# SmoothKen/knn-svc

Measured on AMD Instinct MI355X. Metric: audio-sec converted/sec (xRT) end-to-end, cold target pool, higher is better.
Workload: dtype f32; 1 GPU; north-star point per rank: 30 s source vs 10 min target pool (20 x 30 s), ckpt_type=mix, post_opt_0.2, cold (pool encoded inside the step); seeded random weights of WavLM-Large (6 layers executed) and the 22.9 M-param generator; nq=1500, np_per_rank=30000, wavlm_batch_chunks=32, pipeline_depth=2

## Files before the change

### knn_svc_amd/csrc/common.h

```cpp
#pragma once
#include <hip/hip_runtime.h>
#include <stdint.h>
#include <stdio.h>
#include <stdarg.h>
#include "../../include/knnsvc_hip.h"

typedef float f32x4 __attribute__((ext_vector_type(4)));
typedef float f32x16 __attribute__((ext_vector_type(16)));

extern thread_local char g_knnsvc_err[512];

static inline int knnsvc_fail(int code, const char* fmt, ...) {
    va_list ap;
    va_start(ap, fmt);
    vsnprintf(g_knnsvc_err, sizeof(g_knnsvc_err), fmt, ap);
    va_end(ap);
    return code;
}

#define KN_REQUIRE(cond, ...) do { if (!(cond)) return knnsvc_fail(KNNSVC_EINVAL, __VA_ARGS__); } while (0)

static inline int knnsvc_check_launch(const char* what) {
    hipError_t e = hipGetLastError();
    if (e != hipSuccess) return knnsvc_fail(KNNSVC_EHIP, "%s: %s", what, hipGetErrorString(e));
// ... 30 lines not shown
    if (n_voices < 2 || n_voices > KNNSVC_BLEND_MAX_VOICES)
        return knnsvc_fail(KNNSVC_EINVAL, "%s: n_voices %d outside 2..%d", entry, (int)n_voices, KNNSVC_BLEND_MAX_VOICES);
    if (!host_weights) return knnsvc_fail(KNNSVC_EINVAL, "%s: null weight table", entry);
    out->nv = n_voices;
    for (int s = 0; s < KNNSVC_MAX_SEGMENTS; ++s)
        for (int v = 0; v < KNNSVC_BLEND_MAX_VOICES; ++v) out->w[s][v] = 0.0;
    for (int s = 0; s < n_seg; ++s) {
        double sum = 0.0;
        bool positive = false;
        for (int v = 0; v < n_voices; ++v) {
            const double a = host_weights[(size_t)s * n_voices + v];
            if (!(a >= 0.0 && a <= 1.79769313486231570815e308))
                return knnsvc_fail(KNNSVC_EINVAL, "%s: segment %d: weight %d is %g, not finite and >= 0", entry, s, v, a);
            positive = positive || a > 0.0;
            sum += a;
            out->w[s][v] = a;
        }
        if (!positive) return knnsvc_fail(KNNSVC_EINVAL, "%s: segment %d: no positive weight", entry, s);
        if (!(sum - 1.0 <= 1e-6 && 1.0 - sum <= 1e-6))
            return knnsvc_fail(KNNSVC_EINVAL, "%s: segment %d: the weights sum to %.9g, not 1 (the caller normalises)", entry, s, sum);
    }
    return KNNSVC_OK;
}

struct KnBlendRow { double w[KNNSVC_BLEND_MAX_VOICES]; int live; };
__device__ __forceinline__ KnBlendRow kn_blend_row(const KnBlendWeights& bw, int s) {
    KnBlendRow r;
    r.live = 0;
#pragma unroll
    for (int v = 0; v < KNNSVC_BLEND_MAX_VOICES; ++v) {
        r.w[v] = v < bw.nv ? bw.w[s][v] : 0.0;
        if (r.w[v] != 0.0) ++r.live;
    }
    return r;
}
__device__ __forceinline__ float kn_blend_mix(const KnBlendRow& r, const float (&x)[KNNSVC_BLEND_MAX_VOICES]) {
#pragma clang fp contract(off)
    double acc = 0.0;
    float one = 0.f;
    bool first = true;
#pragma unroll
    for (int v = 0; v < KNNSVC_BLEND_MAX_VOICES; ++v) {
        if (r.w[v] != 0.0) {
            const double p = r.w[v] * (double)x[v];
            acc = first ? p : acc + p;
            first = false;
            one = x[v];
        }
    }
    return r.live == 1 ? one : (float)acc;
}

bool knnsvc_match_generic_k();

template <auto KERNEL>
static inline int kn_lds_optin(int bytes, const char* entry) {
    static int granted = 0;
    if (bytes <= granted) return KNNSVC_OK;
    if (hipFuncSetAttribute((const void*)KERNEL, hipFuncAttributeMaxDynamicSharedMemorySize, bytes) != hipSuccess)
        return knnsvc_fail(KNNSVC_EHIP, "%s: hipFuncSetAttribute failed", entry);
    granted = bytes;
    return KNNSVC_OK;
}

template <int WN, int TM, int TN>
struct Acc32 {
    __device__ __forceinline__ static int acc_row(int wave, int lane, int i, int r) {
        return (wave / WN) * TM * 32 + i * 32 + (r & 3) + 8 * (r >> 2) + 4 * (lane >> 5);
    }
    __device__ __forceinline__ static int acc_col(int wave, int lane, int j) {
        return (wave % WN) * TN * 32 + j * 32 + (lane & 31);
    }
};

#define KN_ZERO_ACC(ACC, TM, TN, NR)                                                                            \
    _Pragma("unroll") for (int i = 0; i < (TM); ++i)                                                           \
        _Pragma("unroll") for (int j = 0; j < (TN); ++j)                                                       \
            _Pragma("unroll") for (int r = 0; r < (NR); ++r) ACC[i][j][r] = 0.f;

namespace {
__global__ __launch_bounds__(256) void kn_zero_kernel(unsigned* __restrict__ p, long n) {
    const long i = (long)blockIdx.x * 256 + threadIdx.x;
    if (i < n) p[i] = 0u;
}
}
static inline int kn_zero_async(void* p, size_t bytes, hipStream_t st) {
    const long n = (long)(bytes / 4);
    if (n == 0) return KNNSVC_OK;
    hipLaunchKernelGGL(kn_zero_kernel, dim3((unsigned)((n + 255) / 256)), dim3(256), 0, st, (unsigned*)p, n);
    return knnsvc_check_launch("zero_fill");
}

__device__ __forceinline__ float kn_gelu(float x) {
#ifdef KN_GELU_ERFF
    return 0.5f * x * (1.0f + erff(x * 0.70710678118654752440f));
#else
#pragma clang fp contract(off)
    const float z = fabsf(x) * 0.70710678118654752440f;
    const float t = __builtin_amdgcn_rcpf(fmaf(0.39f, z, 1.0f));
    float p = -0.1137684788031453f;
    p = fmaf(p, t, 0.4433318425354039f);
    p = fmaf(p, t, -0.3176995829519751f);
    p = fmaf(p, t, 0.32477925011974735f);
    p = fmaf(p, t, 0.045694387408764885f);
    p = fmaf(p, t, 0.11766258084307574f);
    p *= t;
// ... 72 lines not shown
```

### knn_svc_amd/csrc/elementwise.hip

```cpp
#include "common.h"
#include <cstdlib>
#include "gemm2_core.h"

namespace {

__device__ __forceinline__ void store_split4(float* row, int c, f32x4 y) {
    g2_u32x2 hi, lo;
    f16x2_split4(y, KN_F16X2_A_SCALE, hi, lo);
    char* ob = (char*)row + (c >> 5) * 128 + (c & 31) * 2;
    *(g2_u32x2*)ob = hi;
    *(g2_u32x2*)(ob + 64) = lo;
}
__device__ __forceinline__ f32x4 load_split4(const float* row, int c) {
    const char* ib = (const char*)row + (c >> 5) * 128 + (c & 31) * 2;
    const g2_u32x2 hi = *(const g2_u32x2*)ib, lo = *(const g2_u32x2*)(ib + 64);
    f32x4 y;
#pragma unroll
    for (int e = 0; e < 4; ++e) {
        const unsigned short hb = (unsigned short)(hi[e >> 1] >> (16 * (e & 1))), lb = (unsigned short)(lo[e >> 1] >> (16 * (e & 1)));
        y[e] = ((float)__builtin_bit_cast(_Float16, hb) + (float)__builtin_bit_cast(_Float16, lb)) * (1.0f / KN_F16X2_A_SCALE);
    }
    return y;
}

__device__ __forceinline__ float gelu_erf(float v) {
#pragma clang fp contract(off)
    return kn_gelu(v);
}

template <int MAXV, int R>
__global__ __launch_bounds__(256) void layernorm_kernel(const float* __restrict__ x, long rows, int dim, int ldx,
                                                       const float* __restrict__ gamma, const float* __restrict__ beta,
                                                       int gelu, float* __restrict__ out, int ldo) {
#pragma clang fp contract(off)
    const int lane = threadIdx.x & 63;
    const long row0 = ((long)blockIdx.x * 4 + (threadIdx.x >> 6)) * R;
    if (row0 >= rows) return;
    f32x4 v[R][MAXV];
    float s[R];
#pragma unroll
    for (int r = 0; r < R; ++r) {
        s[r] = 0.f;
        const bool ok = row0 + r < rows;
        const float* xr = x + (row0 + r) * (long)ldx;
#pragma unroll
        for (int i = 0; i < MAXV; ++i) {
            const int c = lane * 4 + 256 * i;
            if (ok && c < dim) { v[r][i] = *(const f32x4*)(xr + c); s[r] += (v[r][i][0] + v[r][i][1]) + (v[r][i][2] + v[r][i][3]); }
            else v[r][i] = (f32x4){0.f, 0.f, 0.f, 0.f};
        }
    }
    float mean[R], q[R];
#pragma unroll
    for (int r = 0; r < R; ++r) mean[r] = wave_sum(s[r]) / (float)dim;
#pragma unroll
    for (int r = 0; r < R; ++r) {
        q[r] = 0.f;
#pragma unroll
        for (int i = 0; i < MAXV; ++i) {
            const int c = lane * 4 + 256 * i;
            if (c < dim) {
#pragma unroll
                for (int e = 0; e < 4; ++e) { const float d = v[r][i][e] - mean[r]; q[r] = fmaf(d, d, q[r]); }
            }
        }
    }
#pragma unroll
    for (int r = 0; r < R; ++r) {
        const float var = wave_sum(q[r]) / (float)dim;
        const float rstd = 1.0f / sqrtf(var + 1e-5f);
        if (row0 + r >= rows) continue;
        float* orow = out + (row0 + r) * (long)ldo;
#pragma unroll
        for (int i = 0; i < MAXV; ++i) {
            const int c = lane * 4 + 256 * i;
            if (c < dim) {
                const f32x4 g = *(const f32x4*)(gamma + c), b = *(const f32x4*)(beta + c);
                f32x4 y;
#pragma unroll
                for (int e = 0; e < 4; ++e) {
                    float t = fmaf((v[r][i][e] - mean[r]) * rstd, g[e], b[e]);
                    y[e] = (gelu & 1) ? gelu_erf(t) : t;
                }
                if (gelu & 2) store_split4(orow, c, y);
                else *(f32x4*)(orow + c) = y;
            }
        }
    }
}

template <int CPL, int KMAXT, int RP>
__global__ __launch_bounds__(256) void conv0_ln_gelu_kernel(const float* __restrict__ x, long L, long T, int k, int stride,
                                                           const float* __restrict__ w, const float* __restrict__ gamma,
                                                           const float* __restrict__ beta, float* __restrict__ out, int split, int subs) {
    __shared__ float xs[2][64 * 8 + 32];
    const int lane = threadIdx.x & 63, wave = threadIdx.x >> 6;
    const int C = CPL * 64;
    const long b = blockIdx.y;
    const float* xb = x + b * L;
    const int span = 63 * stride + k;
    constexpr int NP = (CPL + 1) / 2;
    f32x2 wr[NP][KMAXT], g[NP], be[NP];
#pragma unroll
    for (int c = 0; c < NP; ++c) {
        const int ch = lane * CPL + 2 * c, ch1 = CPL > 1 ? ch + 1 : ch;
        g[c] = (f32x2){gamma[ch], gamma[ch1]}; be[c] = (f32x2){beta[ch], beta[ch1]};
#pragma unroll
        for (int t = 0; t < KMAXT; ++t) wr[c][t] = t < k ? (f32x2){w[ch * k + t], w[ch1 * k + t]} : (f32x2){0.f, 0.f};
    }
  for (int sub = 0; sub < subs; ++sub) {
    const long m0 = ((long)blockIdx.x * subs + sub) * 64;
    if (m0 >= T) break;
    float* xsb = xs[sub & 1];
    for (int i = threadIdx.x; i < span; i += 256) {
        const long p = m0 * stride + i;
        xsb[i] = p < L ? xb[p] : 0.f;
    }
    __syncthreads();
    for (int r = 0; r < 16; r += RP) {
        f32x2 y[RP][NP];
        float s[RP], mean[RP], q[RP], rstd[RP];
#pragma unroll
        for (int u = 0; u < RP; ++u) {
            const int lm = wave * 16 + r + u;
            float xv[KMAXT];
#pragma unroll
            for (int t = 0; t < KMAXT; ++t) xv[t] = t < k ? xsb[lm * stride + t] : 0.f;
            s[u] = 0.f;
#pragma unroll
            for (int c = 0; c < NP; ++c) {
                f32x2 a = {0.f, 0.f};
#pragma unroll
                for (int t = 0; t < KMAXT; ++t) a = __builtin_elementwise_fma(wr[c][t], (f32x2)(xv[t]), a);
                y[u][c] = a; s[u] += a[0]; if (CPL > 1) s[u] += a[1];
            }
        }
#pragma unroll
        for (int u = 0; u < RP; ++u) mean[u] = (RP > 1 ? wave_sum_dpp(s[u]) : wave_sum(s[u])) / (float)C;
#pragma unroll
        for (int u = 0; u < RP; ++u) {
            q[u] = 0.f;
#pragma unroll
            for (int c = 0; c < CPL; ++c) { const float d = y[u][c >> 1][c & 1] - mean[u]; q[u] += d * d; }
        }
#pragma unroll
        for (int u = 0; u < RP; ++u) rstd[u] = 1.0f / sqrtf((RP > 1 ? wave_sum_dpp(q[u]) : wave_sum(q[u])) / (float)C + 1e-5f);
#pragma unroll
        for (int u = 0; u < RP; ++u) {
            const long m = m0 + wave * 16 + r + u;
            if (m >= T) break;
            float* o = out + (b * T + m) * C + lane * CPL;
#pragma unroll
            for (int c = 0; c < NP; ++c) y[u][c] = kn_gelu2(__builtin_elementwise_fma((y[u][c] - mean[u]) * rstd[u], g[c], be[c]));
            if (CPL % 4 == 0) {
                if (split) {
                    float* orow = out + (b * T + m) * C;
#pragma unroll
                    for (int c = 0; c < CPL; c += 4) store_split4(orow, lane * CPL + c, (f32x4){y[u][c / 2][0], y[u][c / 2][1], y[u][c / 2 + 1][0], y[u][c / 2 + 1][1]});
                } else {
#pragma unroll
                    for (int c = 0; c < CPL; c += 4) *(f32x4*)(o + c) = (f32x4){y[u][c / 2][0], y[u][c / 2][1], y[u][c / 2 + 1][0], y[u][c / 2 + 1][1]};
                }
            } else {
#pragma unroll
                for (int c = 0; c < CPL; ++c) o[c] = y[u][c >> 1][c & 1];
            }
        }
    }
  }
}

__global__ __launch_bounds__(256) void gate_kernel(const float* __restrict__ xn, long rows, int heads, int ldx,
                                                  const float* __restrict__ w2, const float* __restrict__ b2,
                                                  const float* __restrict__ grep_a, float* __restrict__ gate, int split) {
    const int lane = threadIdx.x & 63;
    const long row = (long)blockIdx.x * 4 + (threadIdx.x >> 6);
    if (row >= rows) return;
    const int h = lane >> 2, part = lane & 3;
    float sa = 0.f, sb = 0.f;
    if (h < heads) {
        const float* xr = xn + row * (long)ldx + lane * 16;
#pragma unroll
        for (int e = 0; e < 16; e += 4) {
            const f32x4 xv = split ? load_split4(xn + row * (long)ldx, lane * 16 + e) : *(const f32x4*)(xr + e);
            const f32x4 wa = *(const f32x4*)(w2 + part * 16 + e), wb = *(const f32x4*)(w2 + 64 + part * 16 + e);
#pragma unroll
            for (int t = 0; t < 4; ++t) { sa += xv[t] * wa[t]; sb += xv[t] * wb[t]; }
        }
    }
    sa += __shfl_xor(sa, 1, 64); sa += __shfl_xor(sa, 2, 64);
    sb += __shfl_xor(sb, 1, 64); sb += __shfl_xor(sb, 2, 64);
    if (h < heads && part == 0) {
        const float ga = 1.0f / (1.0f + expf(-(sa + b2[0])));
        const float gb = 1.0f / (1.0f + expf(-(sb + b2[1])));
        gate[row * heads + h] = ga * (gb * grep_a[h] - 1.0f) + 2.0f;
    }
}

__global__ __launch_bounds__(256) void weighted_gather_kernel(const long* __restrict__ idx, const float* __restrict__ w,
                                                             long nq, int k, const float* __restrict__ pool, int dim,
                                                             int ld, int mean_mode, float* __restrict__ out) {
#pragma clang fp contract(off)
    const long row = blockIdx.x;
    const bool mean = !w && mean_mode == 1;
    for (int c = threadIdx.x; c < dim; c += 256) {
        float acc = 0.f;
        for (int j = 0; j < k; ++j) {
            const float wj = w ? w[row * k + j] : 1.0f / (float)k;
            const float x = pool[idx[row * k + j] * (long)ld + c];
            const float t = mean ? x : x * wj;
            acc = j == 0 ? t : acc + t;
        }
        out[row * (long)dim + c] = mean ? acc / (float)k : acc;
    }
}

__global__ void reflect_pad_kernel(const float* __restrict__ x, long n, int pad, float* __restrict__ out) {
    const long i = (long)blockIdx.x * blockDim.x + threadIdx.x;
    if (i >= n + 2 * (long)pad) return;
    long j = i - pad;
    if (j < 0) j = -j;
    if (j >= n) j = 2 * (n - 1) - j;
// ... 74 lines not shown
    for (int o = 32; o > 0; o >>= 1) mx = fmaxf(mx, __shfl_xor(mx, o, 64));
    const float f = f0[t];
    for (int k = lane + 1; k <= n_harm; k += 64) {
        float v;
        if (f == 0.f) v = k == 1 ? mx : 0.f;
        else {
            const int nb = bins * 8;
            float pos = ((f * (float)k) * 2.0f) * (float)nb / 16000.0f;
            pos = fminf(pos, (float)nb);
            const int gi = (int)rintf(pos);
            if (gi >= nb) v = 0.f;
            else {
                float src = ((float)gi + 0.5f) * 0.125f - 0.5f;
                if (src < 0.f) src = 0.f;
                const int i0 = (int)src;
                const int i1 = i0 + (i0 < bins - 1 ? 1 : 0);
                const float l1 = src - (float)i0, l0 = 1.0f - l1;
                v = l0 * s[i0] + l1 * s[i1];
            }
        }
        harm[t * n_harm + (k - 1)] = 0.0108f * v;
    }
}

__global__ __launch_bounds__(256) void mask_rows_kernel(float* __restrict__ x, int T, int dim, int ld, const int* __restrict__ lens) {
    const int b = blockIdx.y;
    const int len = lens[b];
    const long n4 = (long)(T - len) * (dim / 4);
    for (long i = (long)blockIdx.x * blockDim.x + threadIdx.x; i < n4; i += (long)gridDim.x * blockDim.x) {
        const long r = len + i / (dim / 4); const int c = (int)(i % (dim / 4)) * 4;
        *(f32x4*)(x + ((long)b * T + r) * ld + c) = (f32x4){0.f, 0.f, 0.f, 0.f};
    }
}

}

extern "C" int knnsvc_mask_rows(float* x, int32_t batches, int32_t T, int32_t dim, int32_t ld, const int32_t* lens, void* stream) {
    KN_REQUIRE(x && lens && batches > 0 && batches <= 65535 && T > 0 && dim > 0 && dim % 4 == 0 && ld >= dim && ld % 4 == 0 &&
               ((uintptr_t)x & 15) == 0, "mask_rows: bad arguments");
    hipLaunchKernelGGL(mask_rows_kernel, dim3(64, (unsigned)batches), dim3(256), 0, (hipStream_t)stream, x, T, dim, ld, lens);
    return knnsvc_check_launch("mask_rows");
}

extern "C" int knnsvc_layernorm(const float* x, int64_t rows, int32_t dim, int32_t ldx, const float* gamma,
                                const float* beta, int32_t gelu, float* out, int32_t ldo, void* stream) {
    KN_REQUIRE(x && gamma && beta && out, "layernorm: null pointer");
    KN_REQUIRE(dim > 0 && dim % 4 == 0 && dim <= 2048, "layernorm: dim must be a multiple of 4 and <= 2048");
    KN_REQUIRE(ldx % 4 == 0 && ldo % 4 == 0 && ldx >= dim && ldo >= dim, "layernorm: bad row strides");
    KN_REQUIRE(!(gelu & 2) || (dim % 32 == 0 && ldo % 32 == 0), "layernorm: split output needs dim % 32 == 0 and ldo % 32 == 0");
    KN_REQUIRE(((uintptr_t)x & 15) == 0 && ((uintptr_t)out & 15) == 0 && ((uintptr_t)gamma & 15) == 0 &&
               ((uintptr_t)beta & 15) == 0, "layernorm: pointers must be 16-byte aligned");
    if (rows <= 0) return KNNSVC_OK;
    hipStream_t st = (hipStream_t)stream;
    if (dim <= 512)
        hipLaunchKernelGGL((layernorm_kernel<2, 4>), dim3((unsigned)cdiv64(rows, 16)), dim3(256), 0, st, x, (long)rows, dim, ldx,
                           gamma, beta, gelu, out, ldo);
    else if (dim <= 1024)
        hipLaunchKernelGGL((layernorm_kernel<4, 2>), dim3((unsigned)cdiv64(rows, 8)), dim3(256), 0, st, x, (long)rows, dim, ldx,
                           gamma, beta, gelu, out, ldo);
    else
        hipLaunchKernelGGL((layernorm_kernel<8, 1>), dim3((unsigned)cdiv64(rows, 4)), dim3(256), 0, st, x, (long)rows, dim, ldx,
                           gamma, beta, gelu, out, ldo);
    return knnsvc_check_launch("layernorm");
}

extern "C" int knnsvc_wavlm_gate(const float* xn, int64_t rows, int32_t heads, int32_t head_dim, int32_t ldx,
                                 const float* w2, const float* b2, const float* grep_a, float* gate, int32_t x_f16x2, void* stream) {
    KN_REQUIRE(xn && w2 && b2 && grep_a && gate, "wavlm_gate: null pointer");
    KN_REQUIRE(head_dim == 64 && heads >= 1 && heads <= 16, "wavlm_gate: head_dim must be 64, heads <= 16");
    KN_REQUIRE(ldx % 4 == 0 && ldx >= heads * 64 && ((uintptr_t)xn & 15) == 0 && ((uintptr_t)w2 & 15) == 0,
               "wavlm_gate: alignment");
    if (rows <= 0) return KNNSVC_OK;
    hipLaunchKernelGGL(gate_kernel, dim3((unsigned)cdiv64(rows, 4)), dim3(256), 0, (hipStream_t)stream,
                       xn, (long)rows, heads, ldx, w2, b2, grep_a, gate, x_f16x2);
    return knnsvc_check_launch("wavlm_gate");
}

extern "C" int knnsvc_weighted_gather(const int64_t* idx, const float* w, int64_t nq, int32_t k, const float* pool,
                                      int32_t dim, int32_t ld, int32_t mean_mode, float* out, void* stream) {
    KN_REQUIRE(idx && pool && out && k > 0 && dim > 0 && ld >= dim, "weighted_gather: bad arguments");
    KN_REQUIRE(mean_mode == 0 || mean_mode == 1, "weighted_gather: mean_mode %d is neither 0 nor 1", (int)mean_mode);
    if (nq <= 0) return KNNSVC_OK;
    hipLaunchKernelGGL(weighted_gather_kernel, dim3((unsigned)nq), dim3(256), 0, (hipStream_t)stream,
                       (const long*)idx, w, (long)nq, k, pool, dim, ld, mean_mode, out);
    return knnsvc_check_launch("weighted_gather");
}

extern "C" int knnsvc_reflect_pad(const float* x, int64_t n, int32_t pad, float* out, void* stream) {
    KN_REQUIRE(x && out && n > pad && pad >= 0, "reflect_pad: needs n > pad >= 0");
    const long tot = n + 2 * (long)pad;
    hipLaunchKernelGGL(reflect_pad_kernel, dim3((unsigned)cdiv64(tot, 256)), dim3(256), 0, (hipStream_t)stream,
                       x, (long)n, pad, out);
    return knnsvc_check_launch("reflect_pad");
}

extern "C" int knnsvc_reflect_pad_batch(const float* x, const int64_t* offs, int32_t batches, int32_t pad, float* out,
                                        int64_t stride, void* stream) {
    KN_REQUIRE(x && offs && out && batches > 0 && batches <= 65535 && pad >= 0 && stride > 2 * (int64_t)pad,
               "reflect_pad_batch: bad arguments (every item needs n > pad; stride > 2 pad)");
    const unsigned gx = (unsigned)(cdiv64(stride, 256) < 2048 ? cdiv64(stride, 256) : 2048);
    hipLaunchKernelGGL(reflect_pad_batch_kernel, dim3(gx, (unsigned)batches), dim3(256), 0, (hipStream_t)stream,
                       x, (const long*)offs, pad, out, (long)stride);
    return knnsvc_check_launch("reflect_pad_batch");
}

extern "C" int knnsvc_spec_harm(const float* reim, int64_t rows, int32_t bins, int32_t ld, const float* f0, int32_t n_harm,
                                float* spec, float* harm, void* stream) {
    KN_REQUIRE(reim && f0 && spec && harm && bins > 0 && bins <= 4096 && ld >= 2 * bins && n_harm > 0, "spec_harm: bad arguments");
    if (rows <= 0) return KNNSVC_OK;
    hipLaunchKernelGGL(spec_harm_kernel, dim3((unsigned)cdiv64(rows, 4)), dim3(256), (size_t)4 * bins * sizeof(float),
                       (hipStream_t)stream, reim, (long)rows, bins, ld, f0, n_harm, spec, harm);
    return knnsvc_check_launch("spec_harm");
}

extern "C" int knnsvc_complex_mag(const float* reim, int64_t rows, int32_t bins, int32_t ld, float* out, void* stream) {
    KN_REQUIRE(reim && out && bins > 0 && ld >= 2 * bins, "complex_mag: bad arguments");
    if (rows <= 0) return KNNSVC_OK;
    hipLaunchKernelGGL(complex_mag_kernel, dim3((unsigned)cdiv64(rows * bins, 256)), dim3(256), 0,
                       (hipStream_t)stream, reim, (long)rows, bins, ld, out);
    return knnsvc_check_launch("complex_mag");
}

extern "C" int knnsvc_harmonic_amps(const float* spec, const float* f0, int64_t T, int32_t bins, int32_t n_harm,
                                    float* harm, void* stream) {
    KN_REQUIRE(spec && f0 && harm && bins > 0 && n_harm > 0, "harmonic_amps: bad arguments");
    if (T <= 0) return KNNSVC_OK;
    hipLaunchKernelGGL(harmonic_amps_kernel, dim3((unsigned)cdiv64(T * n_harm, 256)), dim3(256), 0,
                       (hipStream_t)stream, spec, f0, (long)T, bins, n_harm, harm);
    return knnsvc_check_launch("harmonic_amps");
}

extern "C" int knnsvc_wavlm_conv0(const float* x, int32_t batches, int64_t L, const float* w, int32_t channels, int32_t k,
                                  int32_t stride, const float* gamma, const float* beta, float* out, int32_t out_f16x2, void* stream) {
    KN_REQUIRE(x && w && gamma && beta && out, "wavlm_conv0: null pointer");
    KN_REQUIRE(batches > 0 && batches <= 65535 && L >= k && k >= 1 && k <= 16 && stride >= 1 && stride <= 8,
               "wavlm_conv0: needs 1 <= k <= 16, 1 <= stride <= 8");
    KN_REQUIRE(channels == 64 || channels == 128 || channels == 256 || channels == 512, "wavlm_conv0: channels must be 64/128/256/512");
    KN_REQUIRE(!out_f16x2 || channels >= 256, "wavlm_conv0: split output needs >= 256 channels");
    const long T = (L - k) / stride + 1;
    hipStream_t st = (hipStream_t)stream;
    static int rp = -1, subs_env = -1;
    if (rp < 0) { const char* e = getenv("KNNSVC_CONV0_RP"); rp = e ? atoi(e) : 2; if (rp != 1 && rp != 4) rp = 2; }
    if (subs_env < 0) { const char* e = getenv("KNNSVC_CONV0_SUBS"); subs_env = e ? atoi(e) : 8; if (subs_env < 1 || subs_env > 64) subs_env = 8; }
    const int subs = cdiv64(T, 64L * subs_env) * batches >= 3072 ? subs_env : 1;
    dim3 grid((unsigned)cdiv64(T, 64L * subs), (unsigned)batches);
#define KN_C0R(CPL, KM, RP) hipLaunchKernelGGL((conv0_ln_gelu_kernel<CPL, KM, RP>), grid, dim3(256), 0, st, x, (long)L, T, k, stride, w, gamma, beta, out, out_f16x2, subs)
#define KN_C0(CPL, KM) { if (rp == 2) KN_C0R(CPL, KM, 2); else if (rp == 4) KN_C0R(CPL, KM, 4); else KN_C0R(CPL, KM, 1); }
    if (k <= 10) {
        if (channels == 512) KN_C0(8, 10) else if (channels == 256) KN_C0(4, 10) else if (channels == 128) KN_C0(2, 10) else KN_C0(1, 10)
    } else {
        if (channels == 512) KN_C0(8, 16) else if (channels == 256) KN_C0(4, 16) else if (channels == 128) KN_C0(2, 16) else KN_C0(1, 16)
    }
#undef KN_C0R
#undef KN_C0
    return knnsvc_check_launch("wavlm_conv0");
}

namespace {

__global__ __launch_bounds__(256) void round_f16_kernel(const float* __restrict__ x, long n, float* __restrict__ out) {
    const long i = ((long)blockIdx.x * 256 + threadIdx.x) * 4;
    if (i + 3 < n) {
        const f32x4 v = *(const f32x4*)(x + i);
        f32x4 r;
#pragma unroll
        for (int e = 0; e < 4; ++e) r[e] = (float)(_Float16)v[e];
        *(f32x4*)(out + i) = r;
    } else {
        for (long j = i; j < n; ++j) out[j] = (float)(_Float16)x[j];
    }
}

__global__ __launch_bounds__(256) void amp_ratio_kernel(const float* __restrict__ spec_q, int ld_q,
                                                       const float* __restrict__ spec_pool, int ld_pool, long np,
                                                       const long* __restrict__ idx, long nq, int k, int bins,
                                                       float* __restrict__ out) {
    const int lane = threadIdx.x & 63;
    const long t = (long)blockIdx.x * 4 + (threadIdx.x >> 6);
    if (t >= nq) return;
    double s = 0.0;
    for (int c = lane; c < bins; c += 64) s += (double)fabsf(spec_q[t * ld_q + c]);
    const float orig = (float)wave_sum_d(s);
    for (int j = 0; j < k; ++j) {
        long id = idx[t * k + j];
        id = id < 0 ? 0 : (id > np - 1 ? np - 1 : id);
        double a = 0.0;
        for (int c = lane; c < bins; c += 64) a += (double)fabsf(spec_pool[id * ld_pool + c]);
        const float l1 = (float)wave_sum_d(a);
        if (lane == 0) out[t * k + j] = orig / (l1 + 1e-5f);
    }
}

}

extern "C" int knnsvc_round_f16(const float* x, int64_t n, float* out, void* stream) {
    KN_REQUIRE(x && out && n >= 0, "round_f16: bad arguments");
    KN_REQUIRE(((uintptr_t)x & 15) == 0 && ((uintptr_t)out & 15) == 0, "round_f16: pointers must be 16-byte aligned");
    if (n == 0) return KNNSVC_OK;
    hipLaunchKernelGGL(round_f16_kernel, dim3((unsigned)cdiv64(n, 1024)), dim3(256), 0, (hipStream_t)stream, x, (long)n, out);
    return knnsvc_check_launch("round_f16");
}

extern "C" int knnsvc_amp_ratio(const float* spec_q, int32_t ld_q, const float* spec_pool, int32_t ld_pool, int64_t np,
                                const int64_t* idx, int64_t nq, int32_t k, int32_t bins, float* out, void* stream) {
    KN_REQUIRE(spec_q && spec_pool && idx && out, "amp_ratio: null pointer");
    KN_REQUIRE(np > 0 && k > 0 && bins > 0 && ld_q >= bins && ld_pool >= bins, "amp_ratio: bad sizes");
// ... 6 lines not shown
```

### knn_svc_amd/csrc/models.hip

```cpp
#include <stdlib.h>
#include <string.h>
#include <vector>
#include "common.h"

namespace {

constexpr size_t SLOT_FLOATS = 64 * 32;

__global__ __launch_bounds__(256) void zero_fill_kernel(f32x4* __restrict__ p, long n4) {
    const long i = (long)blockIdx.x * 256 + threadIdx.x;
    if (i < n4) p[i] = (f32x4){0.f, 0.f, 0.f, 0.f};
}
int zero_slots(float* p, size_t floats, void* st) {
    const long n4 = (long)(floats / 4);
    hipLaunchKernelGGL(zero_fill_kernel, dim3((unsigned)((n4 + 255) / 256)), dim3(256), 0, (hipStream_t)st, (f32x4*)p, n4);
    return knnsvc_check_launch("zero_slots");
}

struct WavLM {
    knnsvc_wavlm_desc d;
    std::vector<knnsvc_wavlm_conv> conv;
    std::vector<knnsvc_wavlm_layer> layers;
    std::vector<float> mix;
};
// ... 14 lines not shown
        if (n < c.k) return 0;
        n = (n - c.k) / c.stride + 1;
    }
    return n;
}

knnsvc_conv_desc base_desc() {
    knnsvc_conv_desc c;
    memset(&c, 0, sizeof(c));
    c.taps = 1; c.stride = 1; c.dil = 1; c.a_slope = 1.0f; c.div = 1.0f; c.batches = 1; c.groups = 1;
    return c;
}
void set_w(knnsvc_conv_desc& c, const knnsvc_weight& w) { c.w = w.w; c.w_f16x2 = w.w_f16x2; c.w_f16x2_scale = w.w_f16x2 ? w.w_f16x2_scale : 0.f; }

int linear(const float* x, const knnsvc_weight& w, const float* bias, float* out, int64_t M, int N, int K, int act, const float* resid,
           bool x_split, int out_split, const float* x_absmax, float* out_absmax, void* st) {
    knnsvc_conv_desc c = base_desc();
    c.x = x; c.ldx = K; c.t_in = (int32_t)M; c.cin = K; set_w(c, w); c.n = N; c.bias = bias; c.out = out; c.ldo = N; c.m = (int32_t)M;
    c.act = act; c.resid = resid; c.ldr = resid ? N : 0; c.x_f16x2 = x_split ? 1 : 0; c.out_f16x2 = out_split;
    c.x_absmax = x_absmax; c.out_absmax = out_absmax;
    return knnsvc_conv_gemm(&c, st);
}

int encode(const WavLM& m, const float* wav, int B, int64_t L, const int32_t* lens, const float* table, float* out, Arena& ar, void* st) {
    const bool run = ar.base != nullptr;
    const knnsvc_wavlm_desc& d = m.d;
    const int E = d.E, H = d.H;
    const int n_slots = 2 + (int)m.conv.size() + 4 * d.n_layers;
    float* slots = ar.f((size_t)n_slots * SLOT_FLOATS);
    int next_slot = 0, rc0 = 0;
    if (run && (rc0 = zero_slots(slots, (size_t)n_slots * SLOT_FLOATS, st)) != 0) return rc0;
    auto new_slot = [&]() -> float* { float* s = run ? slots + (size_t)next_slot * SLOT_FLOATS : nullptr; ++next_slot; return s; };
    auto slot_of = [&](const float* x, int64_t rows, int cols, int ld, float*& s) -> int {
        s = new_slot();
        return run ? knnsvc_absmax(x, rows, cols, ld, s, st) : 0;
    };
    int rc = 0;
#define KN_RUN(CALL) do { if (run) { rc = (CALL); if (rc) return rc; } } while (0)

    const float* x = wav;
    int64_t t_in = L; int cin = 1;
    bool x_sp = false;
    size_t need[2] = {0, 0};
    {
        int64_t t = L;
        for (size_t li = 0; li < m.conv.size(); ++li) {
            KN_REQUIRE(t >= m.conv[li].k, "wavlm_encode: chunk shorter than the extractor's receptive field");
            t = (t - m.conv[li].k) / m.conv[li].stride + 1;
            const size_t fl = (size_t)B * t * m.conv[li].dim;
            need[li & 1] = fl > need[li & 1] ? fl : need[li & 1];
        }
    }
    float* pp[2] = {ar.f(need[0]), ar.f(need[1])};
    for (size_t li = 0; li < m.conv.size(); ++li) {
        const knnsvc_wavlm_conv& c = m.conv[li];
        const int64_t t_out = (t_in - c.k) / c.stride + 1;
        KN_REQUIRE(t_out > 0, "wavlm_encode: chunk shorter than the extractor's receptive field");
        float* y = pp[li & 1];
        const bool fused0 = li == 0 && cin == 1 && (c.dim == 64 || c.dim == 128 || c.dim == 256 || c.dim == 512) && c.k <= 16 && c.stride <= 8;
        if (fused0) {
            x_sp = c.out_split && c.dim % 32 == 0 && c.dim >= 256 && m.conv.size() > 1;
            KN_RUN(knnsvc_wavlm_conv0(x, B, t_in, c.w.w, c.dim, c.k, c.stride, c.ln_g, c.ln_b, y, x_sp ? 1 : 0, st));
        } else {
            float* xs = nullptr;
            if (!x_sp && cin % 32 == 0) { rc = slot_of(x, (int64_t)B * t_in, cin, cin, xs); if (rc) return rc; }
            knnsvc_conv_desc g = base_desc();
            g.x = x; g.x_bstride = t_in * cin; g.ldx = cin; g.t_in = (int32_t)t_in; g.cin = cin; g.taps = c.k; g.stride = c.stride;
            set_w(g, c.w); g.n = c.dim; g.out = y; g.o_bstride = t_out * c.dim; g.ldo = c.dim; g.m = (int32_t)t_out; g.batches = B;
            g.x_f16x2 = x_sp ? 1 : 0; g.x_absmax = xs;
            KN_RUN(knnsvc_conv_gemm(&g, st));
            x_sp = c.out_split && c.dim % 32 == 0 && li + 1 < m.conv.size();
            KN_RUN(knnsvc_layernorm(y, (int64_t)B * t_out, c.dim, c.dim, c.ln_g, c.ln_b, 1 | (x_sp ? 2 : 0), y, c.dim, st));
        }
        x = y; t_in = t_out; cin = c.dim;
    }
    const int64_t T = t_in, R = (int64_t)B * T;
    KN_REQUIRE(!x_sp && R * (int64_t)(d.ffn > 3 * E ? d.ffn : 3 * E) < (1ll << 31), "wavlm_encode: batch too large");
    const bool f_sp = d.feats_split && cin % 32 == 0;
    float* feats = ar.f((size_t)R * cin);
    KN_RUN(knnsvc_layernorm(x, R, cin, cin, d.ln_g, d.ln_b, f_sp ? 2 : 0, feats, cin, st));
    float* fs = nullptr;
    if (!f_sp) { rc = slot_of(feats, R, cin, cin, fs); if (rc) return rc; }
    float* x_slot = d.pos_a_scale > 0.f ? nullptr : new_slot();
    float* xa = ar.f((size_t)R * E);
    float* xb = ar.f((size_t)R * E);
    KN_RUN(linear(feats, d.proj, d.proj_b, xa, R, E, cin, KNNSVC_ACT_NONE, nullptr, f_sp, 0, fs, x_slot, st));
    if (lens) KN_RUN(knnsvc_mask_rows(xa, B, (int32_t)T, E, E, lens, st));
    {
        const int G = d.pos_groups, K = d.pos_k, cg = E / G;
        knnsvc_conv_desc g = base_desc();
        g.x = xa; g.x_bstride = T * E; g.x_gstride = cg; g.ldx = E; g.t_in = (int32_t)T; g.cin = cg; g.taps = K; g.pad = K / 2;
        set_w(g, d.pos); g.w_gstride = (int64_t)cg * cg * K; g.n = cg; g.bias = d.pos_b; g.bias_gstride = cg;
        g.out = xb; g.o_bstride = T * E; g.o_gstride = cg; g.ldo = E; g.m = (int32_t)T; g.act = KNNSVC_ACT_GELU;
        g.resid = xa; g.r_bstride = T * E; g.r_gstride = cg; g.ldr = E; g.batches = B; g.groups = G;
        g.x_absmax = x_slot; g.a_f16x2_scale = d.pos_a_scale;
        KN_RUN(knnsvc_conv_gemm(&g, st));
    }
    float* cur = xb;
    float* spare[2] = {xa, ar.f((size_t)R * E)};
    float* acc = nullptr;
    const bool mixed = !m.mix.empty();
    if (mixed) {
        acc = ar.f((size_t)R * E);
        KN_RUN(knnsvc_axpy(cur, R * E, m.mix[0], 0, acc, st));
    }
    float* xn = ar.f((size_t)R * E);
    float* gate = ar.f((size_t)R * H);
    float* qkv = ar.f((size_t)R * 3 * E);
    float* att = ar.f((size_t)R * E);
    float* hmid = ar.f((size_t)R * d.ffn);
    for (int l = 0; l < d.n_layers; ++l) {
        const knnsvc_wavlm_layer& ly = m.layers[l];
        const bool last = l == d.n_layers - 1;
        const bool e_sp = ly.xn_split && E % 32 == 0;
        KN_RUN(knnsvc_layernorm(cur, R, E, E, ly.ln1_g, ly.ln1_b, e_sp ? 2 : 0, xn, E, st));
        KN_RUN(knnsvc_wavlm_gate(xn, R, H, 64, E, ly.gate_w, ly.gate_b, ly.grep_a, gate, e_sp ? 1 : 0, st));
        const bool narrow = ly.attn_f16 != 0;
        const bool kv_sp = E % 32 == 0 && narrow;
        float* s1 = nullptr;
        if (!e_sp) { rc = slot_of(xn, R, E, E, s1); if (rc) return rc; }
        KN_RUN(linear(xn, ly.wqkv, ly.bqkv, qkv, R, 3 * E, E, KNNSVC_ACT_NONE, nullptr, e_sp, kv_sp ? E : 0, s1, nullptr, st));
        const bool a_sp = E % 32 == 0 && narrow;
        KN_RUN(knnsvc_wavlm_attention(qkv, gate, table, B, (int32_t)T, H, att, (a_sp ? 1 : 0) | (narrow ? 0 : 4), kv_sp ? 1 : 0, lens, st));
        float* s2 = nullptr;
        if (!a_sp) { rc = slot_of(att, R, E, E, s2); if (rc) return rc; }
        float* x1 = spare[0];
        KN_RUN(linear(att, ly.wo, ly.bo, x1, R, E, E, KNNSVC_ACT_NONE, cur, a_sp, 0, s2, nullptr, st));
        const bool e2_sp = ly.xn2_split && E % 32 == 0;
        KN_RUN(knnsvc_layernorm(x1, R, E, E, ly.ln2_g, ly.ln2_b, e2_sp ? 2 : 0, xn, E, st));
        const bool h_sp = ly.h_split && d.ffn % 32 == 0;
        float* h_slot = h_sp ? nullptr : new_slot();
        float* s3 = nullptr;
        if (!e2_sp) { rc = slot_of(xn, R, E, E, s3); if (rc) return rc; }
// ... 287 lines not shown
```

Before: 928.1 x real-time.

## Precompute conv0 LayerNorm stats via weight covariance Cholesky; fuse final conv LN with feature LN

The first conv's LayerNorm mean and variance are now derived analytically from the input window, using the per-tap weight means and a Cholesky factor of the weight covariance computed once per block in double precision. This removes the per-row cross-lane reductions, and each wave now owns its own 64-row tile with a private LDS buffer. The last conv layer's LN+GELU is also fused with the feature-projection LayerNorm into a single two-pass kernel, saving one full read/write of the feature tensor and one launch. The trade-offs are extra per-block setup work, changed launch bounds and subs heuristics, and numerics that differ slightly from the direct computation.

New measurement: 931.1 x real-time (median of 6 runs). About the same (+0.3%).

```diff
diff --git a/knn_svc_amd/csrc/common.h b/knn_svc_amd/csrc/common.h
--- a/knn_svc_amd/csrc/common.h
+++ b/knn_svc_amd/csrc/common.h
@@ -106,6 +106,9 @@
 }
 
 bool knnsvc_match_generic_k();
+
+int kn_layernorm_twice(const float* x, int64_t rows, int32_t dim, int32_t ldx, const float* gamma, const float* beta, int32_t gelu,
+                       const float* gamma2, const float* beta2, int32_t flags2, float* out, int32_t ldo, void* stream);
 
 template <auto KERNEL>
 static inline int kn_lds_optin(int bytes, const char* entry) {
diff --git a/knn_svc_amd/csrc/elementwise.hip b/knn_svc_amd/csrc/elementwise.hip
--- a/knn_svc_amd/csrc/elementwise.hip
+++ b/knn_svc_amd/csrc/elementwise.hip
@@ -28,10 +28,11 @@
     return kn_gelu(v);
 }
 
-template <int MAXV, int R>
+template <int MAXV, int R, bool TWO>
 __global__ __launch_bounds__(256) void layernorm_kernel(const float* __restrict__ x, long rows, int dim, int ldx,
-                                                       const float* __restrict__ gamma, const float* __restrict__ beta,
-                                                       int gelu, float* __restrict__ out, int ldo) {
+                                                       const float* __restrict__ gamma, const float* __restrict__ beta, int gelu,
+                                                       const float* __restrict__ gamma2, const float* __restrict__ beta2, int gelu2,
+                                                       float* __restrict__ out, int ldo) {
 #pragma clang fp contract(off)
     const int lane = threadIdx.x & 63;
     const long row0 = ((long)blockIdx.x * 4 + (threadIdx.x >> 6)) * R;
@@ -50,51 +51,83 @@
             else v[r][i] = (f32x4){0.f, 0.f, 0.f, 0.f};
         }
     }
-    float mean[R], q[R];
-#pragma unroll
-    for (int r = 0; r < R; ++r) mean[r] = wave_sum(s[r]) / (float)dim;
-#pragma unroll
-    for (int r = 0; r < R; ++r) {
-        q[r] = 0.f;
-#pragma unroll
-        for (int i = 0; i < MAXV; ++i) {
-            const int c = lane * 4 + 256 * i;
-            if (c < dim) {
-#pragma unroll
-                for (int e = 0; e < 4; ++e) { const float d = v[r][i][e] - mean[r]; q[r] = fmaf(d, d, q[r]); }
-            }
-        }
-    }
-#pragma unroll
-    for (int r = 0; r < R; ++r) {
-        const float var = wave_sum(q[r]) / (float)dim;
-        const float rstd = 1.0f / sqrtf(var + 1e-5f);
-        if (row0 + r >= rows) continue;
-        float* orow = out + (row0 + r) * (long)ldo;
-#pragma unroll
-        for (int i = 0; i < MAXV; ++i) {
-            const int c = lane * 4 + 256 * i;
-            if (c < dim) {
-                const f32x4 g = *(const f32x4*)(gamma + c), b = *(const f32x4*)(beta + c);
-                f32x4 y;
-#pragma unroll
-                for (int e = 0; e < 4; ++e) {
-                    float t = fmaf((v[r][i][e] - mean[r]) * rstd, g[e], b[e]);
-                    y[e] = (gelu & 1) ? gelu_erf(t) : t;
+#pragma unroll
+    for (int pass = 0; pass < (TWO ? 2 : 1); ++pass) {
+        const bool last = pass == (TWO ? 1 : 0);
+        const float* __restrict__ gm = pass ? gamma2 : gamma;
+        const float* __restrict__ bt = pass ? beta2 : beta;
+        const int fl = pass ? gelu2 : gelu;
+        if (pass) {
+#pragma unroll
+            for (int r = 0; r < R; ++r) {
+                s[r] = 0.f;
+                const bool ok = row0 + r < rows;
+#pragma unroll
+                for (int i = 0; i < MAXV; ++i)
+                    if (ok && lane * 4 + 256 * i < dim) s[r] += (v[r][i][0] + v[r][i][1]) + (v[r][i][2] + v[r][i][3]);
+            }
+        }
+        float mean[R], q[R];
+#pragma unroll
+        for (int r = 0; r < R; ++r) mean[r] = wave_sum(s[r]) / (float)dim;
+#pragma unroll
+        for (int r = 0; r < R; ++r) {
+            q[r] = 0.f;
+#pragma unroll
+            for (int i = 0; i < MAXV; ++i) {
+                const int c = lane * 4 + 256 * i;
+                if (c < dim) {
+#pragma unroll
+                    for (int e = 0; e < 4; ++e) { const float d = v[r][i][e] - mean[r]; q[r] = fmaf(d, d, q[r]); }
                 }
-                if (gelu & 2) store_split4(orow, c, y);
-                else *(f32x4*)(orow + c) = y;
-            }
-        }
-    }
-}
-
+            }
+        }
+#pragma unroll
+        for (int r = 0; r < R; ++r) {
+            const float var = wave_sum(q[r]) / (float)dim;
+            const float rstd = 1.0f / sqrtf(var + 1e-5f);
+            if (row0 + r >= rows) continue;
+            float* orow = out + (row0 + r) * (long)ldo;
+#pragma unroll
+            for (int i = 0; i < MAXV; ++i) {
+                const int c = lane * 4 + 256 * i;
+                if (c < dim) {
+                    const f32x4 g = *(const f32x4*)(gm + c), b = *(const f32x4*)(bt + c);
+                    f32x4 y;
+#pragma unroll
+                    for (int e = 0; e < 4; ++e) {
+                        float t = fmaf((v[r][i][e] - mean[r]) * rstd, g[e], b[e]);
+                        y[e] = (fl & 1) ? gelu_erf(t) : t;
+                    }
+                    if (!last) v[r][i] = y;
+                    else if (fl & 2) store_split4(orow, c, y);
+                    else *(f32x4*)(orow + c) = y;
+                }
+            }
+        }
+    }
+}
+
+__device__ __forceinline__ double lane_bcast_d(double v, int src) {
+    const long b = __builtin_bit_cast(long, v);
+    const int lo = __builtin_amdgcn_readlane((int)b, src), hi = __builtin_amdgcn_readlane((int)(b >> 32), src);
+    return __builtin_bit_cast(double, ((long)hi << 32) | (unsigned)lo);
+}
+
+#ifndef KN_C0_WAVES
+#define KN_C0_WAVES 3
+#endif
 template <int CPL, int KMAXT, int RP>
-__global__ __launch_bounds__(256) void conv0_ln_gelu_kernel(const float* __restrict__ x, long L, long T, int k, int stride,
+__global__ __launch_bounds__(256, (CPL * KMAXT <= 80 ? KN_C0_WAVES : 2)) void conv0_ln_gelu_kernel(const float* __restrict__ x, long L, long T, int k, int stride,
                                                            const float* __restrict__ w, const float* __restrict__ gamma,
                                                            const float* __restrict__ beta, float* __restrict__ out, int split, int subs) {
-    __shared__ float xs[2][64 * 8 + 32];
-    const int lane = threadIdx.x & 63, wave = threadIdx.x >> 6;
+#pragma clang fp contract(off)
+    constexpr int NJ = KMAXT * (KMAXT + 1) / 2;
+    __shared__ float xs[4][64 * 8 + 32];
+    __shared__ double cm[NJ];
+    __shared__ double wb[KMAXT];
+    __shared__ double lf[KMAXT * KMAXT];
+    const int lane = threadIdx.x & 63, wave = __builtin_amdgcn_readfirstlane(threadIdx.x >> 6);
     const int C = CPL * 64;
     const long b = blockIdx.y;
     const float* xb = x + b * L;
@@ -104,70 +137,129 @@
 #pragma unroll
     for (int c = 0; c < NP; ++c) {
         const int ch = lane * CPL + 2 * c, ch1 = CPL > 1 ? ch + 1 : ch;
+#pragma unroll
+        for (int t = 0; t < KMAXT; ++t) wr[c][t] = t < k ? (f32x2){w[ch * k + t], w[ch1 * k + t]} : (f32x2){0.f, 0.f};
+    }
+    double wm[KMAXT];
+#pragma unroll
+    for (int t = 0; t < KMAXT; ++t) {
+        double a = 0.0;
+#pragma unroll
+        for (int c = 0; c < CPL; ++c) a += (double)wr[c >> 1][t][c & 1];
+        wm[t] = wave_sum_d_dpp(a) / (double)C;
+        if (wave == 0 && lane == 0) wb[t] = wm[t];
+    }
+#pragma unroll
+    for (int a = 0, job = 0; a < KMAXT; ++a) {
+#pragma unroll
+        for (int bb = 0; bb <= a; ++bb, ++job) {
+            if ((job & 3) != wave) continue;
+            double p = 0.0;
+#pragma unroll
+            for (int c = 0; c < CPL; ++c) {
+                float wa = wr[c >> 1][a][c & 1], wc = wr[c >> 1][bb][c & 1];
+                asm volatile("" : "+v"(wa), "+v"(wc));
+                p = __builtin_fma((double)wa - wm[a], (double)wc - wm[bb], p);
+            }
+            p = wave_sum_d_dpp(p) / (double)C;
+            if (lane == 0) cm[job] = p;
+        }
+    }
+    __syncthreads();
+    if (wave == 0) {
+        const int li = lane < KMAXT ? lane : KMAXT - 1;
+        double lr[KMAXT];
+#pragma unroll
+        for (int j = 0; j < KMAXT; ++j) {
+            double s = li >= j ? cm[li * (li + 1) / 2 + j] : 0.0;
+#pragma unroll
+            for (int p = 0; p < j; ++p) s = __builtin_fma(-lr[p], lane_bcast_d(lr[p], j), s);
+            const double d = lane_bcast_d(s, j);
+            const double inv = d > cm[j * (j + 1) / 2 + j] * 0x1p-40 ? 1.0 / __builtin_sqrt(d) : 0.0;
+            lr[j] = li >= j ? s * inv : 0.0;
+        }
+        if (lane < KMAXT) {
+#pragma unroll
+            for (int j = 0; j < KMAXT; ++j) lf[j * KMAXT + lane] = lr[j];
+        }
+    }
+    __syncthreads();
+#pragma unroll
+    for (int c = 0; c < NP; ++c) {
+        const int ch = lane * CPL + 2 * c, ch1 = CPL > 1 ? ch + 1 : ch;
         g[c] = (f32x2){gamma[ch], gamma[ch1]}; be[c] = (f32x2){beta[ch], beta[ch1]};
-#pragma unroll
-        for (int t = 0; t < KMAXT; ++t) wr[c][t] = t < k ? (f32x2){w[ch * k + t], w[ch1 * k + t]} : (f32x2){0.f, 0.f};
-    }
-  for (int sub = 0; sub < subs; ++sub) {
-    const long m0 = ((long)blockIdx.x * subs + sub) * 64;
-    if (m0 >= T) break;
-    float* xsb = xs[sub & 1];
-    for (int i = threadIdx.x; i < span; i += 256) {
-        const long p = m0 * stride + i;
-        xsb[i] = p < L ? xb[p] : 0.f;
-    }
-    __syncthreads();
-    for (int r = 0; r < 16; r += RP) {
-        f32x2 y[RP][NP];
-        float s[RP], mean[RP], q[RP], rstd[RP];
-#pragma unroll
-        for (int u = 0; u < RP; ++u) {
-            const int lm = wave * 16 + r + u;
-            float xv[KMAXT];
-#pragma unroll
-            for (int t = 0; t < KMAXT; ++t) xv[t] = t < k ? xsb[lm * stride + t] : 0.f;
-            s[u] = 0.f;
-#pragma unroll
-            for (int c = 0; c < NP; ++c) {
-                f32x2 a = {0.f, 0.f};
-#pragma unroll
-                for (int t = 0; t < KMAXT; ++t) a = __builtin_elementwise_fma(wr[c][t], (f32x2)(xv[t]), a);
-                y[u][c] = a; s[u] += a[0]; if (CPL > 1) s[u] += a[1];
-            }
-        }
-#pragma unroll
-        for (int u = 0; u < RP; ++u) mean[u] = (RP > 1 ? wave_sum_dpp(s[u]) : wave_sum(s[u])) / (float)C;
-#pragma unroll
-        for (int u = 0; u < RP; ++u) {
-            q[u] = 0.f;
-#pragma unroll
-            for (int c = 0; c < CPL; ++c) { const float d = y[u][c >> 1][c & 1] - mean[u]; q[u] += d * d; }
-        }
-#pragma unroll
-        for (int u = 0; u < RP; ++u) rstd[u] = 1.0f / sqrtf((RP > 1 ? wave_sum_dpp(q[u]) : wave_sum(q[u])) / (float)C + 1e-5f);
-#pragma unroll
-        for (int u = 0; u < RP; ++u) {
-            const long m = m0 + wave * 16 + r + u;
-            if (m >= T) break;
-            float* o = out + (b * T + m) * C + lane * CPL;
-#pragma unroll
-            for (int c = 0; c < NP; ++c) y[u][c] = kn_gelu2(__builtin_elementwise_fma((y[u][c] - mean[u]) * rstd[u], g[c], be[c]));
-            if (CPL % 4 == 0) {
-                if (split) {
-                    float* orow = out + (b * T + m) * C;
-#pragma unroll
-                    for (int c = 0; c < CPL; c += 4) store_split4(orow, lane * CPL + c, (f32x4){y[u][c / 2][0], y[u][c / 2][1], y[u][c / 2 + 1][0], y[u][c / 2 + 1][1]});
+    }
+    float* xw = xs[wave];
+    for (int sub = 0; sub < subs; ++sub) {
+        const long m0 = (((long)blockIdx.x * 4 + wave) * subs + sub) * 64;
+        if (m0 >= T) break;
+        __builtin_amdgcn_fence(__ATOMIC_ACQ_REL, "wavefront");
+        for (int i = lane; i < span; i += 64) {
+            const long p = m0 * stride + i;
+            xw[i] = p < L ? xb[p] : 0.f;
+        }
+        __builtin_amdgcn_fence(__ATOMIC_ACQ_REL, "wavefront");
+        float rs, mu;
+        {
+            double xl[KMAXT];
+#pragma unroll
+            for (int t = 0; t < KMAXT; ++t) xl[t] = t < k ? (double)xw[lane * stride + t] : 0.0;
+            double var = 0.0, mean = 0.0;
+#pragma unroll
+            for (int t = 0; t < KMAXT; ++t) mean = __builtin_fma(wb[t], xl[t], mean);
+            mu = (float)mean;
+#pragma unroll
+            for (int j = 0; j < KMAXT; ++j) {
+                double u = 0.0;
+#pragma unroll
+                for (int i = j; i < KMAXT; ++i) u = __builtin_fma(lf[j * KMAXT + i], xl[i], u);
+                var = __builtin_fma(u, u, var);
+            }
+            rs = 1.0f / sqrtf((float)var + 1e-5f);
+        }
+        const int nrow = T - m0 < 64 ? (int)(T - m0) : 64;
+        for (int r = 0; r < nrow; r += RP) {
+            f32x2 y[RP][NP];
+            float rr[RP], mm[RP];
+#pragma unroll
+            for (int u = 0; u < RP; ++u) {
+                const int lm = r + u;
+                float xv[KMAXT];
+#pragma unroll
+                for (int t = 0; t < KMAXT; ++t) xv[t] = t < k ? xw[lm * stride + t] : 0.f;
+#pragma unroll
+                for (int c = 0; c < NP; ++c) {
+                    f32x2 a = {0.f, 0.f};
+#pragma unroll
+                    for (int t = 0; t < KMAXT; ++t) a = __builtin_elementwise_fma(wr[c][t], (f32x2)(xv[t]), a);
+                    y[u][c] = a;
+                }
+                rr[u] = __builtin_bit_cast(float, __builtin_amdgcn_readlane(__builtin_bit_cast(int, rs), lm));
+                mm[u] = __builtin_bit_cast(float, __builtin_amdgcn_readlane(__builtin_bit_cast(int, mu), lm));
+            }
+#pragma unroll
+            for (int u = 0; u < RP; ++u) {
+                const long m = m0 + r + u;
+                if (m >= T) break;
+                float* o = out + (b * T + m) * C + lane * CPL;
+#pragma unroll
+                for (int c = 0; c < NP; ++c) y[u][c] = kn_gelu2(__builtin_elementwise_fma((y[u][c] - mm[u]) * rr[u], g[c], be[c]));
+                if (CPL % 4 == 0) {
+                    if (split) {
+                        float* orow = out + (b * T + m) * C;
+#pragma unroll
+                        for (int c = 0; c < CPL; c += 4) store_split4(orow, lane * CPL + c, (f32x4){y[u][c / 2][0], y[u][c / 2][1], y[u][c / 2 + 1][0], y[u][c / 2 + 1][1]});
+                    } else {
+#pragma unroll
+                        for (int c = 0; c < CPL; c += 4) *(f32x4*)(o + c) = (f32x4){y[u][c / 2][0], y[u][c / 2][1], y[u][c / 2 + 1][0], y[u][c / 2 + 1][1]};
+                    }
                 } else {
 #pragma unroll
-                    for (int c = 0; c < CPL; c += 4) *(f32x4*)(o + c) = (f32x4){y[u][c / 2][0], y[u][c / 2][1], y[u][c / 2 + 1][0], y[u][c / 2 + 1][1]};
+                    for (int c = 0; c < CPL; ++c) o[c] = y[u][c >> 1][c & 1];
                 }
-            } else {
-#pragma unroll
-                for (int c = 0; c < CPL; ++c) o[c] = y[u][c >> 1][c & 1];
-            }
-        }
-    }
-  }
+            }
+        }
+    }
 }
 
 __global__ __launch_bounds__(256) void gate_kernel(const float* __restrict__ xn, long rows, int heads, int ldx,
@@ -348,16 +440,31 @@
                ((uintptr_t)beta & 15) == 0, "layernorm: pointers must be 16-byte aligned");
     if (rows <= 0) return KNNSVC_OK;
     hipStream_t st = (hipStream_t)stream;
+    const float* none = nullptr;
     if (dim <= 512)
-        hipLaunchKernelGGL((layernorm_kernel<2, 4>), dim3((unsigned)cdiv64(rows, 16)), dim3(256), 0, st, x, (long)rows, dim, ldx,
-                           gamma, beta, gelu, out, ldo);
+        hipLaunchKernelGGL((layernorm_kernel<2, 4, false>), dim3((unsigned)cdiv64(rows, 16)), dim3(256), 0, st, x, (long)rows, dim, ldx,
+                           gamma, beta, gelu, none, none, 0, out, ldo);
     else if (dim <= 1024)
-        hipLaunchKernelGGL((layernorm_kernel<4, 2>), dim3((unsigned)cdiv64(rows, 8)), dim3(256), 0, st, x, (long)rows, dim, ldx,
-                           gamma, beta, gelu, out, ldo);
+        hipLaunchKernelGGL((layernorm_kernel<4, 2, false>), dim3((unsigned)cdiv64(rows, 8)), dim3(256), 0, st, x, (long)rows, dim, ldx,
+                           gamma, beta, gelu, none, none, 0, out, ldo);
     else
-        hipLaunchKernelGGL((layernorm_kernel<8, 1>), dim3((unsigned)cdiv64(rows, 4)), dim3(256), 0, st, x, (long)rows, dim, ldx,
-                           gamma, beta, gelu, out, ldo);
+        hipLaunchKernelGGL((layernorm_kernel<8, 1, false>), dim3((unsigned)cdiv64(rows, 4)), dim3(256), 0, st, x, (long)rows, dim, ldx,
+                           gamma, beta, gelu, none, none, 0, out, ldo);
     return knnsvc_check_launch("layernorm");
+}
+
+int kn_layernorm_twice(const float* x, int64_t rows, int32_t dim, int32_t ldx, const float* gamma, const float* beta, int32_t gelu,
+                       const float* gamma2, const float* beta2, int32_t flags2, float* out, int32_t ldo, void* stream) {
+    KN_REQUIRE(x && gamma && beta && gamma2 && beta2 && out, "layernorm_twice: null pointer");
+    KN_REQUIRE(dim > 0 && dim % 4 == 0 && dim <= 512 && !(gelu & 2), "layernorm_twice: dim must be a multiple of 4 and <= 512, the first result fp32");
+    KN_REQUIRE(ldx % 4 == 0 && ldo % 4 == 0 && ldx >= dim && ldo >= dim, "layernorm_twice: bad row strides");
+    KN_REQUIRE(!(flags2 & 2) || (dim % 32 == 0 && ldo % 32 == 0), "layernorm_twice: split output needs dim % 32 == 0 and ldo % 32 == 0");
+    KN_REQUIRE(((uintptr_t)x & 15) == 0 && ((uintptr_t)out & 15) == 0 && ((uintptr_t)gamma & 15) == 0 && ((uintptr_t)beta & 15) == 0 &&
+               ((uintptr_t)gamma2 & 15) == 0 && ((uintptr_t)beta2 & 15) == 0, "layernorm_twice: pointers must be 16-byte aligned");
+    if (rows <= 0) return KNNSVC_OK;
+    hipLaunchKernelGGL((layernorm_kernel<2, 4, true>), dim3((unsigned)cdiv64(rows, 16)), dim3(256), 0, (hipStream_t)stream, x, (long)rows, dim,
+                       ldx, gamma, beta, gelu, gamma2, beta2, flags2, out, ldo);
+    return knnsvc_check_launch("layernorm_twice");
 }
 
 extern "C" int knnsvc_wavlm_gate(const float* xn, int64_t rows, int32_t heads, int32_t head_dim, int32_t ldx,
@@ -426,6 +533,7 @@
     return knnsvc_check_launch("harmonic_amps");
 }
 
+static constexpr int KN_C0_SUBS = 4;
 extern "C" int knnsvc_wavlm_conv0(const float* x, int32_t batches, int64_t L, const float* w, int32_t channels, int32_t k,
                                   int32_t stride, const float* gamma, const float* beta, float* out, int32_t out_f16x2, void* stream) {
     KN_REQUIRE(x && w && gamma && beta && out, "wavlm_conv0: null pointer");
@@ -435,19 +543,17 @@
     KN_REQUIRE(!out_f16x2 || channels >= 256, "wavlm_conv0: split output needs >= 256 channels");
     const long T = (L - k) / stride + 1;
     hipStream_t st = (hipStream_t)stream;
-    static int rp = -1, subs_env = -1;
-    if (rp < 0) { const char* e = getenv("KNNSVC_CONV0_RP"); rp = e ? atoi(e) : 2; if (rp != 1 && rp != 4) rp = 2; }
-    if (subs_env < 0) { const char* e = getenv("KNNSVC_CONV0_SUBS"); subs_env = e ? atoi(e) : 8; if (subs_env < 1 || subs_env > 64) subs_env = 8; }
-    const int subs = cdiv64(T, 64L * subs_env) * batches >= 3072 ? subs_env : 1;
-    dim3 grid((unsigned)cdiv64(T, 64L * subs), (unsigned)batches);
-#define KN_C0R(CPL, KM, RP) hipLaunchKernelGGL((conv0_ln_gelu_kernel<CPL, KM, RP>), grid, dim3(256), 0, st, x, (long)L, T, k, stride, w, gamma, beta, out, out_f16x2, subs)
-#define KN_C0(CPL, KM) { if (rp == 2) KN_C0R(CPL, KM, 2); else if (rp == 4) KN_C0R(CPL, KM, 4); else KN_C0R(CPL, KM, 1); }
+    static int subs_env = -1;
+    if (subs_env < 0) { const char* e = getenv("KNNSVC_CONV0_SUBS"); subs_env = e ? atoi(e) : 0; if (subs_env < 1 || subs_env > 64) subs_env = 0; }
+    int subs = subs_env ? subs_env : KN_C0_SUBS;
+    while (!subs_env && subs > 1 && cdiv64(T, 256L * subs) * batches < 1536) subs >>= 1;
+    dim3 grid((unsigned)cdiv64(T, 256L * subs), (unsigned)batches);
+#define KN_C0(CPL, KM) hipLaunchKernelGGL((conv0_ln_gelu_kernel<CPL, KM, 2>), grid, dim3(256), 0, st, x, (long)L, T, k, stride, w, gamma, beta, out, out_f16x2, subs);
     if (k <= 10) {
         if (channels == 512) KN_C0(8, 10) else if (channels == 256) KN_C0(4, 10) else if (channels == 128) KN_C0(2, 10) else KN_C0(1, 10)
     } else {
         if (channels == 512) KN_C0(8, 16) else if (channels == 256) KN_C0(4, 16) else if (channels == 128) KN_C0(2, 16) else KN_C0(1, 16)
     }
-#undef KN_C0R
 #undef KN_C0
     return knnsvc_check_launch("wavlm_conv0");
 }
diff --git a/knn_svc_amd/csrc/models.hip b/knn_svc_amd/csrc/models.hip
--- a/knn_svc_amd/csrc/models.hip
+++ b/knn_svc_amd/csrc/models.hip
@@ -90,6 +90,7 @@
         }
     }
     float* pp[2] = {ar.f(need[0]), ar.f(need[1])};
+    bool tail2 = false;
     for (size_t li = 0; li < m.conv.size(); ++li) {
         const knnsvc_wavlm_conv& c = m.conv[li];
         const int64_t t_out = (t_in - c.k) / c.stride + 1;
@@ -108,7 +109,8 @@
             g.x_f16x2 = x_sp ? 1 : 0; g.x_absmax = xs;
             KN_RUN(knnsvc_conv_gemm(&g, st));
             x_sp = c.out_split && c.dim % 32 == 0 && li + 1 < m.conv.size();
-            KN_RUN(knnsvc_layernorm(y, (int64_t)B * t_out, c.dim, c.dim, c.ln_g, c.ln_b, 1 | (x_sp ? 2 : 0), y, c.dim, st));
+            tail2 = li + 1 == m.conv.size() && c.dim <= 512;
+            if (!tail2) KN_RUN(knnsvc_layernorm(y, (int64_t)B * t_out, c.dim, c.dim, c.ln_g, c.ln_b, 1 | (x_sp ? 2 : 0), y, c.dim, st));
         }
         x = y; t_in = t_out; cin = c.dim;
     }
@@ -116,7 +118,8 @@
     KN_REQUIRE(!x_sp && R * (int64_t)(d.ffn > 3 * E ? d.ffn : 3 * E) < (1ll << 31), "wavlm_encode: batch too large");
     const bool f_sp = d.feats_split && cin % 32 == 0;
     float* feats = ar.f((size_t)R * cin);
-    KN_RUN(knnsvc_layernorm(x, R, cin, cin, d.ln_g, d.ln_b, f_sp ? 2 : 0, feats, cin, st));
+    if (tail2) KN_RUN(kn_layernorm_twice(x, R, cin, cin, m.conv.back().ln_g, m.conv.back().ln_b, 1, d.ln_g, d.ln_b, f_sp ? 2 : 0, feats, cin, st));
+    else KN_RUN(knnsvc_layernorm(x, R, cin, cin, d.ln_g, d.ln_b, f_sp ? 2 : 0, feats, cin, st));
     float* fs = nullptr;
     if (!f_sp) { rc = slot_of(feats, R, cin, cin, fs); if (rc) return rc; }
     float* x_slot = d.pos_a_scale > 0.f ? nullptr : new_slot();
```
